# conradludgate/rustyguard

Hardware: AMD Instinct MI355X
Metric: GiB/s + Mpkt/s device-resident ChaCha20-Poly1305 seal/open, 1/2/4/8 MI355X (higher is better)
Workload: dtype u32; 1 GPU; cfg2: 64 Ki packets x 1500 B, one session key, seal then open, 1 MI355X; packets_per_gpu=65536, payload_bytes_per_packet=1504, wire_bytes_per_gpu=100663296, sessions=1, parallelism=split1 (no collective), split=1, wg_per_cu=auto

## Files before the change

rustyguard_amd/csrc/rg_internal.h:

```cpp
#pragma once
#include <hip/hip_ext.h>
#include <hip/hip_runtime.h>
#include <stdint.h>

#include "../../include/rg_aead.h"

namespace rg {

constexpr uint32_t kMaxPayload = 1u << 20;

struct SealArgs {
    const uint32_t *keys;
    const uint32_t *receivers;
    const rg_pkt_desc *desc;
    const uint64_t *counters;
    uint8_t *buf;
    uint64_t buf_len;
    uint8_t *status;
    uint64_t *dbg;
    uint32_t nkeys;
    uint32_t n;
};

struct OpenArgs {
    const uint32_t *keys;
    const rg_pkt_desc *desc;
    uint8_t *buf;
    uint64_t buf_len;
    uint8_t *status;
    uint64_t *counters_out;
    uint64_t *dbg;
    uint32_t nkeys;
    uint32_t n;
};

struct MacArgs {
    const uint32_t *keys;
    uint32_t key_len;
    uint32_t nkeys;
    uint32_t which;
    uint32_t n;
    const rg_pkt_desc *desc;
    const uint8_t *buf;
    uint64_t buf_len;
    uint8_t *status;
    uint32_t *key_out;
    uint32_t *key_state;
};
hipError_t launch_mac_verify(const MacArgs &a, hipStream_t s);

struct WorkspaceCursor {
    uint64_t at = 0;
    uint64_t take(uint64_t bytes) {
        const uint64_t o = at;
        at += (bytes + 255) & ~255ull;
        return o;
    }
    uint64_t total() const { return at ? at : 256; }
};

constexpr uint32_t kReplayTile = 2048;
struct ReplayLayout {
    uint64_t rdesc;
    uint64_t hash;
    uint64_t order[2];
    uint64_t hist;
    uint64_t agg_val;
    uint64_t agg_flag;
    uint64_t lf;
    uint64_t ctr;
    uint64_t widx;
    uint64_t undo;
    uint64_t ustatus;
    uint64_t udesc;
    uint64_t total;
    uint64_t hash_cap;
    uint32_t nblk;
    uint32_t passes;
};
inline ReplayLayout replay_layout(uint64_t n, uint32_t nwin) {
    ReplayLayout L{};
    if (n > 0xFFFFFFFFull) return L;
    WorkspaceCursor ws;
    L.hash_cap = 64;
    while (L.hash_cap < 2 * n) L.hash_cap <<= 1;
    L.nblk = (uint32_t)((n + kReplayTile - 1) / kReplayTile);
    for (uint32_t top = nwin ? nwin - 1 : 0; top; top >>= 8) ++L.passes;
    L.rdesc = ws.take(n * sizeof(rg_pkt_desc));
    L.hash = ws.take(L.hash_cap * 4);
    L.order[0] = ws.take(L.passes > 0 ? n * 4 : 0);
    L.order[1] = ws.take(L.passes > 1 ? n * 4 : 0);
    L.hist = ws.take(L.passes > 0 ? 256ull * L.nblk * 4 : 0);
    L.agg_val = ws.take((uint64_t)L.nblk * 8);
    L.agg_flag = ws.take((uint64_t)L.nblk * 4);
    L.lf = ws.take(n * 8);
    L.ctr = ws.take(n * 8);
    L.widx = ws.take(n * 4);
    L.undo = ws.take(n);
    L.ustatus = ws.take(n);
    L.udesc = ws.take(n * sizeof(rg_pkt_desc));
    L.total = ws.total();
    return L;
}

struct DeviceGuard {
    int dev = -1;
    DeviceGuard() { (void)hipGetDevice(&dev); }
    ~DeviceGuard() {
        if (dev >= 0) (void)hipSetDevice(dev);
    }
    DeviceGuard(const DeviceGuard &) = delete;
    DeviceGuard &operator=(const DeviceGuard &) = delete;
};

struct GeneralJob {
    uint32_t key[8];
    uint32_t nonce[3];
    uint32_t decrypt;
    uint32_t xchacha;
    uint32_t hnonce[4];
    uint64_t aad_off;
    uint64_t aad_len;
    uint64_t payload_off;
    uint64_t payload_len;
    uint64_t tag_off;
    uint32_t status;
    uint32_t pad_;
};

struct Launch {
    int lanes;
    int cus;
    int wg_per_cu;
    int debug_mode;
    int staged_g;
    hipEvent_t done;
};

#define RG_LAUNCH(done, kernel, grid, block, lds, stream, ...)                                              \
    do {                                                                                                   \
        if (done) hipExtLaunchKernelGGL(kernel, grid, block, lds, stream, nullptr, done, 0u, __VA_ARGS__); \
        else hipLaunchKernelGGL(kernel, grid, block, lds, stream, __VA_ARGS__);                            \
    } while (0)
constexpr uint32_t kLdsPerCu = 160u * 1024u;

constexpr uint32_t kClasses = 37;
__host__ __device__ __forceinline__ uint32_t class_hi(uint32_t c) {
    if (c <= 16) return c;
    const uint32_t j = c - 17;
    return (j & 1u) ? (1u << (j / 2 + 5)) : (3u << (j / 2 + 3));
}
__device__ __forceinline__ uint32_t class_of(uint32_t chunks) {
    if (chunks <= 16) return chunks;
    uint32_t c = 17;
    while (c < kClasses - 1 && class_hi(c) < chunks) ++c;
    return c;
}

struct TilePlan {
    const uint32_t *counts;
    const uint32_t *lists;
    uint32_t cap;
    uint32_t target_lanes;
    uint32_t fixed_k;
    uint32_t *classes_out;
    uint32_t *sched;
    uint32_t simds;
    uint32_t *gq;
};

hipError_t launch_plan(const rg_pkt_desc *desc, uint32_t n, bool open, const TilePlan &tp, hipStream_t s);
hipError_t launch_tiles(const SealArgs *sa, const OpenArgs *oa, int G, const TilePlan &tp, const Launch &L,
                        hipStream_t s);
hipError_t prepare_tile_kernels();
constexpr uint32_t kSchedWords = 128;
constexpr uint32_t kSchedStart = 4, kSchedLg = 44, kSchedCnt = 84;
static_assert(kSchedCnt + kClasses <= kSchedWords, "schedule words");

constexpr int kTargets = 6;
__device__ __forceinline__ void schedule_classes(uint32_t *counts, uint32_t *sched, uint32_t simds,
                                                 uint32_t *classes_out) {
    __shared__ uint32_t s_lg[kTargets][64], s_start[kTargets][64], s_est[kTargets], s_total[kTargets];
    __shared__ float s_sum[kTargets];
    const uint32_t c = threadIdx.x & 63, v = threadIdx.x >> 6;
    const uint32_t cnt =
        c < kClasses ? __hip_atomic_load(&counts[c], __ATOMIC_RELAXED, __HIP_MEMORY_SCOPE_AGENT) : 0;
    const uint32_t chunks = c < kClasses ? class_hi(c) : 0;
    const uint64_t used = __ballot(cnt > 0);
    float work = 0.0f;
    for (uint64_t m = used; m; m &= m - 1) {
        const int j = __ffsll((unsigned long long)m) - 1;
        work += (float)(uint32_t)__builtin_amdgcn_readlane((int)cnt, j) * (float)(1 + class_hi((uint32_t)j));
    }
    const uint32_t S = simds ? simds : 1;
    const float mean = work / (64.0f * (float)S);
    constexpr float kF[kTargets] = {1.0f, 1.25f, 1.5f, 2.0f, 3.0f, 0.0f};
    for (uint32_t k = v; k < (uint32_t)kTargets; k += 4) {
        const float tf = kF[k] > 0.0f ? ceilf(mean * kF[k]) : 65535.0f;
        const uint32_t target = tf < 2.0f ? 2u : tf > 65535.0f ? 65535u : (uint32_t)tf;
        uint32_t lg = 0;
        while (lg < 6 && 1 + ((chunks + (1u << lg) - 1) >> lg) > target) ++lg;
        const uint32_t tiles = cnt ? (uint32_t)((((uint64_t)cnt << lg) + 63) >> 6) : 0;
        const uint32_t w = cnt ? 1 + ((chunks + (1u << lg) - 1) >> lg) + (lg ? 1 : 0) : 0;
        uint32_t start = 0, total = 0;
        float sum = 0.0f;
        for (uint64_t m = used; m; m &= m - 1) {
            const int j = __ffsll((unsigned long long)m) - 1;
            const uint32_t wj = (uint32_t)__builtin_amdgcn_readlane((int)w, j);
            const uint32_t tj = (uint32_t)__builtin_amdgcn_readlane((int)tiles, j);
            if (wj > w || (wj == w && (uint32_t)j > c)) start += tj;
            total += tj;
            sum += (float)tj * (float)wj;
        }
        uint32_t est0 = 0, est1 = 0;
        for (uint32_t t = 0, m = 0; t < total; t += S, ++m) {
            const uint32_t a = t + (m & 1u ? S - 1 : 0), b = t + (m & 1u ? 0 : S - 1);
            const uint64_t ha = __ballot(tiles > 0 && start <= a && a < start + tiles);
            const uint64_t hb = __ballot(tiles > 0 && start <= b && b < start + tiles);
            if (ha) est0 += (uint32_t)__builtin_amdgcn_readlane((int)w, __ffsll((unsigned long long)ha) - 1);
            if (hb) est1 += (uint32_t)__builtin_amdgcn_readlane((int)w, __ffsll((unsigned long long)hb) - 1);
        }
        const uint32_t est = est0 > est1 ? est0 : est1;
        s_lg[k][c] = lg;
        s_start[k][c] = start;
        if (c == 0) {
            s_est[k] = est;
            s_sum[k] = sum;
            s_total[k] = total;
        }
    }
    __syncthreads();
    if (v != 0) return;
    uint32_t best = 0;
    for (uint32_t k = 1; k < (uint32_t)kTargets; ++k)
        if (s_est[k] < s_est[best] || (s_est[k] == s_est[best] && s_sum[k] < s_sum[best])) best = k;
    if (c < kClasses) {
        __hip_atomic_store(&counts[c], 0u, __ATOMIC_RELAXED, __HIP_MEMORY_SCOPE_AGENT);
        sched[kSchedStart + c] = s_start[best][c];
        sched[kSchedLg + c] = s_lg[best][c];
        sched[kSchedCnt + c] = cnt;
    }
    if (c == 0) {
        sched[2] = s_total[best];
        if (classes_out) *reinterpret_cast<volatile uint32_t *>(classes_out) = (uint32_t)__popcll(used);
    }
}

struct PipePlan {
    uint32_t *counts;
    const uint32_t *lists;
    uint32_t cap;
    uint32_t *sched;
    uint32_t *classes_out;
    uint32_t simds;
};
hipError_t launch_pipe(const SealArgs *sa, const OpenArgs *oa, const Launch &L, const PipePlan *plan,
                       hipStream_t s);

constexpr uint32_t kFlatGroup = 1024;
hipError_t launch_flat(const SealArgs *sa, const OpenArgs *oa, bool balance, uint4 *junk, int cus, hipStream_t s,
                       hipEvent_t done = nullptr);
uint32_t flat_junk_bytes(int cus);
hipError_t prepare_flat_kernels();
hipError_t prepare_pipe_kernels(int max_wg[2]);
hipError_t launch_rx_resolve(const rg_pkt_desc *desc, uint32_t n, const uint8_t *buf, uint64_t buf_len,
                             const rg_rx_entry *table, uint32_t cap, rg_pkt_desc *out, uint32_t *key_out,
                             hipStream_t s);
__host__ __device__ __forceinline__ uint32_t rx_slot(uint32_t receiver, uint32_t cap) {
    return cap > 1 ? (receiver * 0x9E3779B1u) >> (32 - __builtin_ctz(cap)) : 0u;
}
hipError_t launch_general(GeneralJob *jobs, uint32_t njobs, uint8_t *arena, hipStream_t s);
hipError_t launch_bind_keys(const rg_pkt_desc *in, const uint32_t *key_idx, uint32_t n, rg_pkt_desc *out,
                            hipStream_t s);
hipError_t launch_undo_gather(const rg_pkt_desc *rd, const uint64_t *ctr, const uint32_t *idx, uint32_t m,
                              rg_pkt_desc *out, uint64_t *ctr_out, hipStream_t s);
hipError_t launch_synth_fill(const rg_pkt_desc *desc, const uint32_t *inner_len, uint32_t n, uint8_t *buf,
                             uint64_t buf_len, uint64_t seed, hipStream_t s);

constexpr uint32_t kCtlCounts = 0;
constexpr uint32_t kCtlSched = 64;
constexpr uint32_t kCtlPool = 192;
constexpr uint32_t kCtlWords = 256;
static_assert(kCtlCounts + kClasses + 1 <= kCtlSched && kCtlSched + kSchedWords <= kCtlPool &&
                  kCtlPool + 33 <= kCtlWords, "control block layout");
hipError_t launch_preset(uint8_t *status, uint32_t n, uint32_t *ctl, uint32_t done_init, uint32_t pool_init,
                         hipStream_t s);

}
```

rustyguard_amd/csrc/rg_pipe.hip:

```cpp
#include "rg_device.h"
#include "rg_internal.h"

namespace rg {

struct Chunk {
    uint4 q0, q1, q2, q3;
};

constexpr int kDepth = 3;

typedef unsigned v4u __attribute__((ext_vector_type(4)));
template <int NT> __device__ __forceinline__ uint4 ld16(const uint4 *p) {
    if constexpr (NT & 1) {
        const v4u v = __builtin_nontemporal_load(reinterpret_cast<const v4u *>(p));
        return make_uint4(v.x, v.y, v.z, v.w);
    } else return *p;
}
template <int NT> __device__ __forceinline__ void st16(uint4 *p, const uint4 &x) {
    if constexpr (NT & 4) return;
    else if constexpr (NT & 2) {
        const v4u v = {x.x, x.y, x.z, x.w};
        __builtin_nontemporal_store(v, reinterpret_cast<v4u *>(p));
    } else *p = x;
}
template <int MODE> constexpr int mode_nt() { return MODE == 7 ? 4 : (MODE >= 4 && MODE <= 6) ? MODE - 3 : 0; }

template <int NT = 0>
__device__ __forceinline__ void load_chunk(Chunk &c, const uint4 *pl, uint32_t t, uint32_t last) {
    const uint32_t b = 4 * t;
    c.q0 = ld16<NT>(pl + min(b + 0, last));
    c.q1 = ld16<NT>(pl + min(b + 1, last));
    c.q2 = ld16<NT>(pl + min(b + 2, last));
    c.q3 = ld16<NT>(pl + min(b + 3, last));
}

__device__ __forceinline__ void absorb_chunk(Acc &h, const Chunk &c, const Mul &r, uint32_t cnt) {
    acc_block_pred(h, c.q0, r, cnt > 0);
    acc_block_pred(h, c.q1, r, cnt > 1);
    acc_block_pred(h, c.q2, r, cnt > 2);
    acc_block_pred(h, c.q3, r, cnt > 3);
}

constexpr uint32_t kPipeLinesFlag = 4u;
constexpr uint32_t kRingBytes = 64u * 256u;
typedef __attribute__((address_space(3))) v4u lds_u4;
__device__ __forceinline__ v4u to_v4(const uint4 &a) { return v4u{a.x, a.y, a.z, a.w}; }
__device__ __forceinline__ uint32_t ring_g(uint32_t p) { return (p & 1u) ^ (((p >> 1) & 1u) * 10u) ^ (((p >> 2) & 1u) * 4u); }

struct Ring {
    lds_u4 *wr;
    lds_u4 *rd;
    uint32_t fo[2][4];
    uint32_t self;
    uint64_t base;
    __amdgpu_buffer_rsrc_t rs;
    uint32_t gw, gr;
};

__device__ __forceinline__ bool frame_window(const uint8_t *frame, uint32_t len, uint64_t &base) {
    const uint64_t f = reinterpret_cast<uint64_t>(frame);
    const uint64_t f0 = uniform_u64(f);
    const int64_t dlt = (int64_t)(f - f0);
    const bool near = dlt > -(int64_t)(1u << 30) && dlt < (int64_t)(1u << 30);
    if (__ballot(!near) != 0) return false;
    const uint32_t v = (uint32_t)(dlt + (int64_t)(1u << 30));
    const uint32_t vmax = lane63(wave_scan_max(v)), vmin = 0x7FFFFFFFu - lane63(wave_scan_max(0x7FFFFFFFu - v));
    if ((uint64_t)(vmax - vmin) + len >= (1ull << 31)) return false;
    base = f0 + (uint64_t)vmin - (1ull << 30);
    return true;
}

__device__ __forceinline__ Ring make_ring(uint8_t *frame, uint64_t base) {
    extern __shared__ __attribute__((aligned(16))) uint8_t pipe_lds[];
    const uint32_t lane = threadIdx.x & 63;
    lds_u4 *lb = (lds_u4 *)(pipe_lds + (threadIdx.x >> 6) * kRingBytes);
    Ring R;
    R.wr = lb + 16 * lane;
    R.gw = ring_g(lane);
    R.rd = lb + 16 * (lane >> 3);
    R.gr = ring_g(lane >> 3);
    R.self = (uint32_t)(reinterpret_cast<uint64_t>(frame) - base);
    R.base = base;
    R.rs = __builtin_amdgcn_make_buffer_rsrc(reinterpret_cast<void *>(base), (short)0, 0x7FFFFFFF, 0x00020000);
#pragma unroll
    for (int h = 0; h < 2; ++h)
#pragma unroll
        for (int q = 0; q < 4; ++q)
            R.fo[h][q] = (uint32_t)__shfl((int)R.self, 32 * h + 8 * q + (int)(lane >> 3)) + 16 * (lane & 7u);
    return R;
}

__device__ __forceinline__ Ring pin_window(const Ring &R) {
    Ring o = R;
    o.base = uniform_u64(R.base);
    o.rs = __builtin_amdgcn_make_buffer_rsrc(reinterpret_cast<void *>(o.base), (short)0, 0x7FFFFFFF, 0x00020000);
    return o;
}

#ifndef RG_TAIL_CP
#define RG_TAIL_CP 0
#endif
constexpr int kTailCp = RG_TAIL_CP;

template <int CP = 0> __device__ __forceinline__ void frame_store(const Ring &R, uint32_t off, const uint4 &x) {
    __builtin_amdgcn_raw_buffer_store_b128(to_v4(x), R.rs, (int)(R.self + off), 0, CP);
}

__device__ __forceinline__ void ring_put(const Ring &R, uint32_t t, const uint4 &a, const uint4 &b, const uint4 &c,
                                         const uint4 &d) {
    const uint32_t sw = (4 * (t & 3u)) ^ R.gw;
    R.wr[sw ^ 0] = to_v4(a);
    R.wr[sw ^ 1] = to_v4(b);
    R.wr[sw ^ 2] = to_v4(c);
    R.wr[sw ^ 3] = to_v4(d);
}

struct Ring4 {
    v4u v[4];
};
__device__ __forceinline__ Ring4 ring_get(const Ring &R, uint32_t k, uint32_t h) {
    const uint32_t lane = threadIdx.x & 63;
    const uint32_t set = (2 * k + ((lane >> 2) & 1u)) & 3u;
    const lds_u4 *r = R.rd + 512 * h + ((4 * set + (lane & 3u)) ^ R.gr);
    Ring4 o;
#pragma unroll
    for (int q = 0; q < 4; ++q) o.v[q] = r[128 * q];
    return o;
}

template <bool MASK = false, int CP = 0>
__device__ __forceinline__ void ring_store(const Ring &R, const Ring4 &x, uint32_t k, uint32_t h, uint32_t nblk = 0) {
    if constexpr (MASK) {
        const uint32_t lane = threadIdx.x & 63;
        if (((lane >> 2) & 1u) && 2 * k + 1 >= nblk) return;
    }
#pragma unroll
    for (int q = 0; q < 4; ++q)
        __builtin_amdgcn_raw_buffer_store_b128(x.v[q], R.rs, (int)((h ? R.fo[1][q] : R.fo[0][q]) + 128 * k), 0, CP);
}

template <bool OPEN, bool ABSORB, bool TAIL, int MODE = 0, bool LINES = false, bool FLUSH = false>
__device__ __forceinline__ void pipe_step(uint4 *pl, const Stream &st, const Mul &r, Acc &h, Chunk &pi, Chunk &buf,
                                          uint4 &prev, bool &have_prev, uint32_t t, uint32_t nb, uint32_t c0,
                                          const Ring &R) {
    uint32_t ks[16];
    static_assert(!FLUSH || (LINES && ABSORB && !TAIL), "flush steps");
    Ring4 fl;
    if constexpr (FLUSH) {
        wave_sync();
        fl = ring_get(R, (t - 2) >> 1, t & 1u);
    }
    if constexpr (MODE == 2) {
#pragma unroll
        for (int i = 0; i < 16; ++i) ks[i] = t * 16 + i;
        h.h0 ^= pi.q0.x ^ pi.q1.y ^ pi.q2.z ^ pi.q3.w;
    } else stream_block_hooked(st, c0 + t + 1, ks, [&](int dr) {
        if constexpr (OPEN) {
            const uint32_t bl = TAIL ? nb & 3u : 4u;
            if (dr == 1) acc_block_pred(h, buf.q0, r, bl > 0);
            if (dr == 3) acc_block_pred(h, buf.q1, r, bl > 1);
            if (dr == 5) acc_block_pred(h, buf.q2, r, bl > 2);
            if (dr == 7) acc_block_pred(h, buf.q3, r, bl > 3);
            if (dr % 2 == 1) pin_acc(h);
        } else if constexpr (ABSORB) {
            if (dr == 1) acc_block(h, pi.q0, r);
            if (dr == 3) acc_block(h, pi.q1, r);
            if (dr == 5) acc_block(h, pi.q2, r);
            if (dr == 7) acc_block(h, pi.q3, r);
            if (dr % 2 == 1) pin_acc(h);
        }
    });
    Chunk x = {xor4(buf.q0, ks + 0), xor4(buf.q1, ks + 4), xor4(buf.q2, ks + 8), xor4(buf.q3, ks + 12)};
    uint4 *dst = pl + 4 * t;
    if constexpr (MODE == 1) {
        pi = x;
        buf.q0.x += t; buf.q1.y ^= t; buf.q2.z += h.h0; buf.q3.w ^= t;
        return;
    }
    constexpr int NT = mode_nt<MODE>();
    if constexpr (LINES && !TAIL) {
        ring_put(R, t, prev, x.q0, x.q1, x.q2);
        if constexpr (FLUSH) ring_store(R, fl, MODE == 8 ? ((t - 2) >> 1) & 1u : (t - 2) >> 1, t & 1u);
        prev = x.q3;
        have_prev = true;
    } else if constexpr (TAIL) {
        const uint32_t cnt = nb & 3u;
        if constexpr (LINES) {
            const uint32_t o = 16 + 64 * t;
            if (have_prev) frame_store<kTailCp>(R, o - 16, prev);
            frame_store<kTailCp>(R, o, x.q0);
            if (cnt > 1) frame_store<kTailCp>(R, o + 16, x.q1);
            if (cnt > 2) frame_store<kTailCp>(R, o + 32, x.q2);
        } else {
            if (have_prev) st16<NT>(dst - 1, prev);
            st16<NT>(dst + 0, x.q0);
            if (cnt > 1) st16<NT>(dst + 1, x.q1);
            if (cnt > 2) st16<NT>(dst + 2, x.q2);
        }
        have_prev = false;
    } else {
        if constexpr (ABSORB) st16<NT>(dst - 1, prev);
        else if (have_prev) st16<NT>(dst - 1, prev);
        st16<NT>(dst + 0, x.q0);
        st16<NT>(dst + 1, x.q1);
        st16<NT>(dst + 2, x.q2);
        prev = x.q3;
        have_prev = true;
    }
    if constexpr (!OPEN) pi = x;
    if constexpr (!TAIL) load_chunk<NT & 1>(buf, pl, t + kDepth, nb - 1);
}

template <bool OPEN, int MODE = 0, bool LINES = false>
__device__ __forceinline__ Acc pipe_pass(uint4 *pl, const Stream &st, const Mul &r, uint32_t nb, uint32_t c0,
                                         Chunk &b0, Chunk &b1, Chunk &b2, uint4 head, bool has_head, const Ring &R0) {
    const Ring R = LINES ? pin_window(R0) : R0;
    const uint32_t F = nb >> 2, bl = nb & 3u;
    Acc h = {0, 0, 0, 0, 0};
    Chunk pi = {};
    uint4 prev = head;
    bool have_prev = has_head;
    uint32_t pending = 0;
    if constexpr (LINES) wave_sync();
    if (F > 0) {
        pipe_step<OPEN, false, false, MODE, LINES>(pl, st, r, h, pi, b0, prev, have_prev, 0, nb, c0, R);
        uint32_t t = 1;
        if constexpr (LINES) {
            if (F > 1) pipe_step<OPEN, true, false, MODE, true>(pl, st, r, h, pi, b1, prev, have_prev, 1, nb, c0, R);
            for (t = 2; t + 2 < F; t += 3) {
                pipe_step<OPEN, true, false, MODE, true, true>(pl, st, r, h, pi, b2, prev, have_prev, t, nb, c0, R);
                pipe_step<OPEN, true, false, MODE, true, true>(pl, st, r, h, pi, b0, prev, have_prev, t + 1, nb, c0, R);
                pipe_step<OPEN, true, false, MODE, true, true>(pl, st, r, h, pi, b1, prev, have_prev, t + 2, nb, c0, R);
            }
            if (t < F) pipe_step<OPEN, true, false, MODE, true, true>(pl, st, r, h, pi, b2, prev, have_prev, t, nb, c0, R);
            if (t + 1 < F)
                pipe_step<OPEN, true, false, MODE, true, true>(pl, st, r, h, pi, b0, prev, have_prev, t + 1, nb, c0, R);
            wave_sync();
            for (uint32_t m = F >= 2 ? F - 2 : 0; m < 2 * ((F + 1) >> 1); ++m)
                ring_store<true, kTailCp>(R, ring_get(R, m >> 1, m & 1u), MODE == 8 ? (m >> 1) & 1u : m >> 1, m & 1u,
                                          F);
        } else {
            for (; t + 2 < F; t += 3) {
                pipe_step<OPEN, true, false, MODE, false>(pl, st, r, h, pi, b1, prev, have_prev, t, nb, c0, R);
                pipe_step<OPEN, true, false, MODE, false>(pl, st, r, h, pi, b2, prev, have_prev, t + 1, nb, c0, R);
                pipe_step<OPEN, true, false, MODE, false>(pl, st, r, h, pi, b0, prev, have_prev, t + 2, nb, c0, R);
            }
            if (t < F) pipe_step<OPEN, true, false, MODE, false>(pl, st, r, h, pi, b1, prev, have_prev, t, nb, c0, R);
            if (t + 1 < F) pipe_step<OPEN, true, false, MODE, false>(pl, st, r, h, pi, b2, prev, have_prev, t + 1, nb, c0, R);
        }
        pending = 4;
    }
    if (bl > 0) {
        const uint32_t k = F % kDepth;
        Chunk bp = {k == 1 ? b1.q0 : k == 2 ? b2.q0 : b0.q0, k == 1 ? b1.q1 : k == 2 ? b2.q1 : b0.q1,
                    k == 1 ? b1.q2 : k == 2 ? b2.q2 : b0.q2, k == 1 ? b1.q3 : k == 2 ? b2.q3 : b0.q3};
        if (F > 0) pipe_step<OPEN, true, true, MODE, LINES>(pl, st, r, h, pi, bp, prev, have_prev, F, nb, c0, R);
        else pipe_step<OPEN, false, true, MODE, LINES>(pl, st, r, h, pi, bp, prev, have_prev, F, nb, c0, R);
        pending = bl;
    }
    if constexpr (LINES) {
        if (have_prev) frame_store<kTailCp>(R, 64 * F, prev);
    } else if (have_prev && MODE != 1) st16<mode_nt<MODE>()>(pl + 4 * F - 1, prev);
    if constexpr (!OPEN) absorb_chunk(h, pi, r, pending);
    return h;
}

__device__ __forceinline__ void pipe_tag(Acc h, const Mul &r, uint32_t P, const uint32_t *s, uint32_t tag[4]) {
    acc_add(h, 0, 0, P, 0, 1);
    acc_mul(h, r);
    acc_finish(h, s[0], s[1], s[2], s[3], tag);
}

struct Seg {
    uint32_t c0, nb, after;
};

__device__ __forceinline__ Seg make_seg(uint32_t nb, uint32_t j, uint32_t G) {
    const uint32_t C = (nb + 3) >> 2, L = (C + G - 1) / G;
    const uint32_t c0 = min(j * L, C), c1 = min(c0 + L, C);
    const uint32_t b0 = min(4 * c0, nb), b1 = min(4 * c1, nb);
    return {c0, b1 - b0, nb - b1};
}

__device__ __forceinline__ uint32_t wave_max_u32(uint32_t v) {
#pragma unroll
    for (int o = 32; o >= 1; o >>= 1) v = max(v, (uint32_t)__shfl_xor((int)v, o));
    return v;
}

__device__ __forceinline__ Acc combine_segments(Acc h, const Mul &r, uint32_t after, uint32_t G) {
    if (G == 1) return h;
    const uint32_t bits = 32 - __clz((int)wave_max_u32(after));
    if (bits > 0) {
        Acc x = {1, 0, 0, 0, 0};
        for (int b = (int)bits - 1; b >= 0; --b) {
            Acc sq = x;
            acc_sqr_gen(sq);
            Acc xr = sq;
            acc_mul(xr, r);
            const bool bit = (after >> b) & 1u;
            x.h0 = bit ? xr.h0 : sq.h0; x.h1 = bit ? xr.h1 : sq.h1; x.h2 = bit ? xr.h2 : sq.h2;
            x.h3 = bit ? xr.h3 : sq.h3; x.h4 = bit ? xr.h4 : sq.h4;
        }
        acc_mul_gen(h, make_gen(x));
    }
    for (uint32_t o = 1; o < G; o <<= 1) {
        Acc other;
        other.h0 = (uint32_t)__shfl_xor((int)h.h0, (int)o);
        other.h1 = (uint32_t)__shfl_xor((int)h.h1, (int)o);
        other.h2 = (uint32_t)__shfl_xor((int)h.h2, (int)o);
        other.h3 = (uint32_t)__shfl_xor((int)h.h3, (int)o);
        other.h4 = (uint32_t)__shfl_xor((int)h.h4, (int)o);
        acc_add_acc(h, other);
        acc_fold(h);
    }
    return h;
}

template <int MODE>
__device__ __forceinline__ void pipe_seal_packet(const SealArgs &a, uint32_t i, const rg_pkt_desc &d, uint32_t j,
                                                 uint32_t G, bool lines_ok) {
    const uint32_t P = d.len;
    const bool valid = d.key_idx < a.nkeys && (P & 15u) == 0 && (d.offset & 15u) == 0 && P <= kMaxPayload &&
                       d.offset <= a.buf_len && P + 32 <= a.buf_len - d.offset;
    bool lines = false;
    if constexpr (MODE == 0 || MODE == 8)
        lines = lines_ok && G == 1 && __ballot(valid && P == uniform_u32(P)) == ~0ull;
    uint64_t wbase = 0;
    if (lines) lines = frame_window(a.buf + d.offset, P + 32, wbase);
    if (!valid) {
        if (a.status && j == 0) a.status[i] = d.key_idx == RG_KEY_SKIP ? RG_PKT_REJECTED : RG_PKT_INVALID;
        return;
    }
    uint8_t *frame = a.buf + d.offset;
    const uint32_t nb = P >> 4;
    const Seg sg = make_seg(nb, j, G);
    uint4 *pl = reinterpret_cast<uint4 *>(frame + 16) + (sg.nb ? 4 * sg.c0 : 0);
    Chunk b0, b1, b2;
    if constexpr (MODE == 1) {
        b0 = {make_uint4(i, 1, 2, 3), make_uint4(4, i, 6, 7), make_uint4(8, 9, i, 11), make_uint4(12, 13, 14, i)};
        b1 = b0;
        b2 = b0;
    } else {
        constexpr int NT = mode_nt<MODE>() & 1;
        load_chunk<NT>(b0, pl, 0, sg.nb ? sg.nb - 1 : 0);
        load_chunk<NT>(b1, pl, 1, sg.nb ? sg.nb - 1 : 0);
        load_chunk<NT>(b2, pl, 2, sg.nb ? sg.nb - 1 : 0);
    }
    const Key8 key = load_key(a.keys, d.key_idx);
    const uint64_t ctr = a.counters[i];
    const uint32_t n1 = (uint32_t)ctr, n2 = (uint32_t)(ctr >> 32);
    const Stream stm = make_stream(key, 0u, n1, n2);
    uint32_t ks[16];
    stream_block(stm, 0, ks);
    const Mul r = make_mul(ks[0], ks[1], ks[2], ks[3]);
    const bool head = a.receivers != nullptr && j == 0;
    uint4 hdr = make_uint4(4u, head ? a.receivers[d.key_idx] : 0u, n1, n2);
    Acc h;
    Ring R{};
    if (lines) {
        if (!head) hdr = *reinterpret_cast<const uint4 *>(frame);
        R = make_ring(frame, wbase);
        h = pipe_pass<false, MODE, true>(pl, stm, r, sg.nb, sg.c0, b0, b1, b2, hdr, true, R);
    } else {
        h = pipe_pass<false, MODE, false>(pl, stm, r, sg.nb, sg.c0, b0, b1, b2, hdr, head, Ring{});
    }
    h = combine_segments(h, r, sg.after, G);
    if (j != 0) return;
    uint32_t tag[4];
    pipe_tag(h, r, P, ks + 4, tag);
    const uint4 tagv = make_uint4(tag[0], tag[1], tag[2], tag[3]);
    if (lines) frame_store<kTailCp>(pin_window(R), 16 + P, tagv);
    else *reinterpret_cast<uint4 *>(frame + 16 + P) = tagv;
    if (a.status) a.status[i] = RG_PKT_OK;
}

__device__ __forceinline__ void pipe_open_packet(const OpenArgs &a, uint32_t i, const rg_pkt_desc &d, uint32_t j,
                                                 uint32_t G, bool lines_ok) {
    const uint32_t W = d.len;
    uint32_t st;
    if (d.key_idx == RG_KEY_SKIP) st = RG_PKT_REJECTED;
    else if ((d.offset & 15u) != 0) st = RG_PKT_UNALIGNED;
    else if (d.key_idx >= a.nkeys || W > kMaxPayload + 32 || d.offset > a.buf_len || W > a.buf_len - d.offset ||
             W < 4)
        st = RG_PKT_INVALID;
    else st = 0xFF;
    uint8_t *frame = a.buf + d.offset;
    const bool desc_ok = st == 0xFF;
    const bool go = desc_ok && W >= 32 && (W & 15u) == 0;
    const uint32_t P = go ? W - 32 : 0;
    const uint32_t nb = P >> 4;
    const Seg sg = make_seg(nb, j, G);
    uint4 *safe = const_cast<uint4 *>(reinterpret_cast<const uint4 *>(a.desc + i));
    uint4 *pl = go ? reinterpret_cast<uint4 *>(frame + 16) + (sg.nb ? 4 * sg.c0 : 0) : safe;
    const uint4 hdr = *(desc_ok ? reinterpret_cast<const uint4 *>(frame) : safe);
    Chunk b0, b1, b2;
    load_chunk(b0, pl, 0, sg.nb ? sg.nb - 1 : 0);
    load_chunk(b1, pl, 1, sg.nb ? sg.nb - 1 : 0);
    load_chunk(b2, pl, 2, sg.nb ? sg.nb - 1 : 0);
    const uint4 want = *(go ? reinterpret_cast<const uint4 *>(frame + 16 + P) : safe);
    const Key8 key = load_key(a.keys, go ? d.key_idx : 0);
    uint64_t ctr = 0;
    if (desc_ok) {
        if (hdr.x != 4u) st = hdr.x - 1u < 3u ? RG_PKT_NOT_DATA : RG_PKT_INVALID;
        else if ((W & 15u) != 0 || W < 16) st = RG_PKT_INVALID;
        else {
            ctr = ((uint64_t)hdr.w << 32) | hdr.z;
            if (W < 32) st = RG_PKT_DECRYPT_ERR;
        }
    }
    bool lines = lines_ok && G == 1 && __ballot(st == 0xFF && W == uniform_u32(W)) == ~0ull;
    uint64_t wbase = 0;
    if (lines) lines = frame_window(frame, W, wbase);
    if (st != 0xFF) {
        if (j == 0) {
            a.status[i] = (uint8_t)st;
            if (a.counters_out) a.counters_out[i] = ctr;
        }
        return;
    }
    const uint32_t n1 = (uint32_t)ctr, n2 = (uint32_t)(ctr >> 32);
    const Stream stm = make_stream(key, 0u, n1, n2);
    uint32_t ks[16];
    stream_block(stm, 0, ks);
    const Mul r = make_mul(ks[0], ks[1], ks[2], ks[3]);
    Acc h;
    Ring Ro{};
    if (lines) Ro = make_ring(frame, wbase);
    if (lines) h = pipe_pass<true, 0, true>(pl, stm, r, sg.nb, sg.c0, b0, b1, b2, hdr, true, Ro);
    else h = pipe_pass<true, 0, false>(pl, stm, r, sg.nb, sg.c0, b0, b1, b2, make_uint4(0, 0, 0, 0), false, Ring{});
    h = combine_segments(h, r, sg.after, G);
    uint32_t tag[4];
    pipe_tag(h, r, P, ks + 4, tag);
    const uint32_t diff = (tag[0] ^ want.x) | (tag[1] ^ want.y) | (tag[2] ^ want.z) | (tag[3] ^ want.w);
    if (__ballot(diff != 0)) {
        wave_sync();
        restore_forged(diff != 0, key, n1, n2, pl, sg.c0, sg.nb);
    }
    if (j == 0) {
        a.status[i] = diff == 0 ? RG_PKT_OK : RG_PKT_DECRYPT_ERR;
        if (a.counters_out) a.counters_out[i] = ctr;
    }
}

#if RG_DIAG
__device__ __forceinline__ void pipe_stamp(uint64_t *dbg, uint64_t t0, uint64_t r0, const uint64_t marks[3]) {
    const uint64_t t1 = __builtin_amdgcn_s_memtime(), r1 = __builtin_amdgcn_s_memrealtime();
    if ((threadIdx.x & 63) == 0) {
        uint64_t *o = dbg + 8ull * (blockIdx.x * (blockDim.x / 64) + threadIdx.x / 64);
        o[0] = t1 - t0;
        o[1] = marks[0] ? marks[0] - r0 : 0;
        o[2] = marks[1] ? marks[1] - r0 : 0;
        o[3] = ((uint64_t)(uint32_t)__builtin_amdgcn_s_getreg(0xF814) << 32) | (uint32_t)__builtin_amdgcn_s_getreg(0xF804);
        o[4] = r0;
        o[5] = marks[2] ? marks[2] - t0 : 0;
        o[6] = 1;
        o[7] = r1 - r0;
    }
}
#endif

template <class Body>
__device__ __forceinline__ void pipe_walk(uint32_t n, uint32_t lg0, const PipePlan &pp, const rg_pkt_desc *desc,
                                          bool stamp, uint64_t marks[3], Body &&body) {
    const uint32_t lane = threadIdx.x & 63;
    const bool planned = pp.counts != nullptr;
    uint32_t my_cnt = 0, my_start = 0, my_lg = 0, my_tiles = 0, S = 1, simd = 0, ntiles = 0;
    uint64_t total, first, stride;
    if (planned) {
        my_cnt = lane < kClasses ? pp.sched[kSchedCnt + lane] : 0;
        my_start = lane < kClasses ? pp.sched[kSchedStart + lane] : 0;
        my_lg = lane < kClasses ? pp.sched[kSchedLg + lane] : 0;
        my_tiles = (uint32_t)((((uint64_t)my_cnt << my_lg) + 63) / 64);
        S = pp.simds ? pp.simds : 1;
        const uint32_t slot = blockIdx.x * (blockDim.x / 64) + threadIdx.x / 64;
        simd = slot % S;
        ntiles = pp.sched[2];
        total = (ntiles + S - 1) / S;
        first = slot / S;
        stride = gridDim.x * (blockDim.x / 64) / S;
    } else {
        total = (uint64_t)n << lg0;
        first = blockIdx.x * 256 + threadIdx.x;
        stride = (uint64_t)gridDim.x * 256;
    }
    struct Unit {
        uint32_t i, j, lg;
        bool live;
    };
    auto locate = [&](uint64_t it, uint32_t &list_pos) -> Unit {
        Unit o;
        list_pos = 0;
        if (planned) {
            const uint32_t tile = (uint32_t)it * S + ((it & 1u) ? S - 1 - simd : simd);
            const uint64_t hit = __ballot(lane < kClasses && my_start <= tile && tile < my_start + my_tiles);
            const uint32_t c = uniform_u32((uint32_t)(__ffsll((unsigned long long)hit) - 1));
            o.lg = uniform_u32((uint32_t)__shfl((int)my_lg, (int)c));
            const uint32_t u = (tile - uniform_u32((uint32_t)__shfl((int)my_start, (int)c))) * 64 + lane;
            const uint32_t p = u >> o.lg;
            o.live = tile < ntiles && p < uniform_u32((uint32_t)__shfl((int)my_cnt, (int)c));
            o.j = u & ((1u << o.lg) - 1);
            list_pos = o.live ? c * pp.cap + p : 0;
            o.i = 0;
        } else {
            o.lg = lg0;
            o.live = it < total;
            o.j = (uint32_t)it & ((1u << lg0) - 1);
            o.i = o.live ? (uint32_t)(it >> lg0) : 0;
        }
        return o;
    };
    if (first >= total) return;
    uint32_t q0, q1;
    Unit cur = locate(first, q0), nxt = locate(first + stride, q1);
    if (planned) {
        cur.i = pp.lists[q0];
        nxt.i = pp.lists[q1];
    }
    rg_pkt_desc dcur = desc[cur.live ? cur.i : 0];
    for (uint64_t it = first; it < total; it += stride) {
        uint32_t q2;
        Unit far = locate(it + 2 * stride, q2);
        if (planned) far.i = pp.lists[q2];
        const rg_pkt_desc dnxt = desc[nxt.live ? nxt.i : 0];
        if (stamp && it == first) marks[2] = __builtin_amdgcn_s_memtime();
        if (cur.live) body(cur.i, dcur, cur.j, 1u << cur.lg);
        if (stamp) {
            const uint64_t now = __builtin_amdgcn_s_memrealtime();
            if (it == first) marks[0] = now;
            else if (it == first + stride) marks[1] = now;
        }
        cur = nxt;
        nxt = far;
        dcur = dnxt;
    }
}

template <int MODE> __global__ __launch_bounds__(256) void pipe_seal_kernel(SealArgs a, uint32_t flags, PipePlan pp) {
    uint64_t marks[3] = {0, 0, 0};
    const bool lines = (flags & kPipeLinesFlag) != 0;
#if RG_DIAG
    const uint64_t t0 = __builtin_amdgcn_s_memtime(), r0 = __builtin_amdgcn_s_memrealtime();
    const bool stamp = a.dbg != nullptr;
#else
    constexpr bool stamp = false;
#endif
    pipe_walk(a.n, flags & 3u, pp, a.desc, stamp, marks, [=](uint32_t i, const rg_pkt_desc &d, uint32_t j, uint32_t G) {
        pipe_seal_packet<MODE>(a, i, d, j, G, lines);
    });
#if RG_DIAG
    if (stamp) pipe_stamp(a.dbg, t0, r0, marks);
#endif
}

__global__ __launch_bounds__(256) void pipe_open_kernel(OpenArgs a, uint32_t flags, PipePlan pp) {
    uint64_t marks[3] = {0, 0, 0};
    const bool lines = (flags & kPipeLinesFlag) != 0;
#if RG_DIAG
    const uint64_t t0 = __builtin_amdgcn_s_memtime(), r0 = __builtin_amdgcn_s_memrealtime();
    const bool stamp = a.dbg != nullptr;
#else
    constexpr bool stamp = false;
#endif
    pipe_walk(a.n, flags & 3u, pp, a.desc, stamp, marks, [=](uint32_t i, const rg_pkt_desc &d, uint32_t j, uint32_t G) {
        pipe_open_packet(a, i, d, j, G, lines);
    });
#if RG_DIAG
    if (stamp) pipe_stamp(a.dbg, t0, r0, marks);
#endif
}

static void pipe_grid(uint64_t units, const Launch &L, uint32_t &blocks, uint32_t &lds) {
    const uint64_t want = (units + 255) / 256;
    const uint64_t cap = (uint64_t)L.cus * (uint64_t)L.wg_per_cu;
    blocks = (uint32_t)(want < cap || cap == 0 ? want : cap);
    lds = L.wg_per_cu > 0 ? (kLdsPerCu / L.wg_per_cu) & ~255u : 0;
}

hipError_t launch_pipe(const SealArgs *sa, const OpenArgs *oa, const Launch &L, const PipePlan *plan,
                       hipStream_t s) {
    const uint32_t n = sa ? sa->n : oa->n;
    if (n == 0) return hipSuccess;
    const uint32_t lg = L.lanes >= 4 ? 2 : L.lanes == 2 ? 1 : 0;
    PipePlan pp{};
    uint32_t blocks, lds;
    if (plan) {
        pp = *plan;
        const uint32_t wg = (uint32_t)(L.wg_per_cu > 0 ? L.wg_per_cu : 1);
        blocks = (uint32_t)(L.cus > 0 ? L.cus : 1) * wg;
        lds = (kLdsPerCu / wg) & ~255u;
        if (pp.simds == 0 || ((uint64_t)blocks * 4) % pp.simds != 0) return hipErrorInvalidValue;
    } else {
        pipe_grid((uint64_t)n << lg, L, blocks, lds);
    }
    const uint32_t fl = lg | (lds >= 4 * kRingBytes ? kPipeLinesFlag : 0u);
    if (oa) {
        RG_LAUNCH(L.done, pipe_open_kernel, dim3(blocks), dim3(256), lds, s, *oa, fl, pp);
        return hipGetLastError();
    }
#if RG_DIAG
    switch (L.debug_mode) {
    case 1: hipLaunchKernelGGL(pipe_seal_kernel<1>, dim3(blocks), dim3(256), lds, s, *sa, fl, pp); return hipGetLastError();
    case 2: hipLaunchKernelGGL(pipe_seal_kernel<2>, dim3(blocks), dim3(256), lds, s, *sa, fl, pp); return hipGetLastError();
    case 4: hipLaunchKernelGGL(pipe_seal_kernel<4>, dim3(blocks), dim3(256), lds, s, *sa, fl, pp); return hipGetLastError();
    case 5: hipLaunchKernelGGL(pipe_seal_kernel<5>, dim3(blocks), dim3(256), lds, s, *sa, fl, pp); return hipGetLastError();
    case 6: hipLaunchKernelGGL(pipe_seal_kernel<6>, dim3(blocks), dim3(256), lds, s, *sa, fl, pp); return hipGetLastError();
    case 7: hipLaunchKernelGGL(pipe_seal_kernel<7>, dim3(blocks), dim3(256), lds, s, *sa, fl, pp); return hipGetLastError();
    case 8: hipLaunchKernelGGL(pipe_seal_kernel<8>, dim3(blocks), dim3(256), lds, s, *sa, fl, pp); return hipGetLastError();
    default: break;
    }
#endif
    RG_LAUNCH(L.done, pipe_seal_kernel<0>, dim3(blocks), dim3(256), lds, s, *sa, fl, pp);
    return hipGetLastError();
}

hipError_t prepare_pipe_kernels(int max_wg[2]) {
    const void *f[2] = {(const void *)pipe_seal_kernel<0>, (const void *)pipe_open_kernel};
    for (int w = 0; w < 2; ++w) {
        hipError_t e = hipFuncSetAttribute(f[w], hipFuncAttributeMaxDynamicSharedMemorySize, (int)kLdsPerCu);
        if (e != hipSuccess) return e;
        int nb = 0;
        e = hipOccupancyMaxActiveBlocksPerMultiprocessor(&nb, f[w], 256, 0);
        if (e != hipSuccess) return e;
        max_wg[w] = nb;
    }
#if RG_DIAG
    const void *d[7] = {(const void *)pipe_seal_kernel<1>, (const void *)pipe_seal_kernel<2>,
                        (const void *)pipe_seal_kernel<4>, (const void *)pipe_seal_kernel<5>,
                        (const void *)pipe_seal_kernel<6>, (const void *)pipe_seal_kernel<7>,
                        (const void *)pipe_seal_kernel<8>};
    for (const void *k : d) {
        hipError_t e = hipFuncSetAttribute(k, hipFuncAttributeMaxDynamicSharedMemorySize, (int)kLdsPerCu);
        if (e != hipSuccess) return e;
    }
#endif
    return hipSuccess;
}

}
```

Baseline: 1385 GiB/s.

## Load frame-aligned 64B blocks including header and tag in the pipe loop

Reindexes the pipelined seal/open loads so each 64-byte chunk is aligned to the frame start rather than the payload start. The 16-byte header and the trailing tag now arrive as part of the prefetched chunks, replacing separate header and tag loads and the carried 'prev' register. Open gets the header and tag from the chunk buffers, using lane shuffles when a packet is split across lanes. The intent is fully aligned line-sized accesses and fewer scattered loads. The cost is more complex index bookkeeping and some extra shuffles.

```diff
diff --git a/rustyguard_amd/csrc/rg_internal.h b/rustyguard_amd/csrc/rg_internal.h
--- a/rustyguard_amd/csrc/rg_internal.h
+++ b/rustyguard_amd/csrc/rg_internal.h
@@ -257,6 +257,22 @@
 hipError_t launch_pipe(const SealArgs *sa, const OpenArgs *oa, const Launch &L, const PipePlan *plan,
                        hipStream_t s);
 
+struct Seg {
+    uint32_t c0, nb, after;
+};
+__host__ __device__ inline Seg make_seg(uint32_t nb, uint32_t j, uint32_t G) {
+    const uint32_t C = (nb + 3) >> 2, L = (C + G - 1) / G;
+    const uint32_t c0 = j * L < C ? j * L : C, c1 = c0 + L < C ? c0 + L : C;
+    const uint32_t b0 = 4 * c0 < nb ? 4 * c0 : nb, b1 = 4 * c1 < nb ? 4 * c1 : nb;
+    return {c0, b1 - b0, nb - b1};
+}
+__host__ __device__ inline uint32_t pipe_piece(uint32_t blk, uint32_t i, uint32_t hi) {
+    const uint32_t p = 4 * blk + i;
+    return p < hi ? p : hi;
+}
+__host__ __device__ inline uint32_t pipe_full_steps(uint32_t nb) { return nb >> 2; }
+__host__ __device__ inline uint32_t pipe_last_blocks(uint32_t nb) { return nb & 3u; }
+
 constexpr uint32_t kFlatGroup = 1024;
 hipError_t launch_flat(const SealArgs *sa, const OpenArgs *oa, bool balance, uint4 *junk, int cus, hipStream_t s,
                        hipEvent_t done = nullptr);
diff --git a/rustyguard_amd/csrc/rg_pipe.hip b/rustyguard_amd/csrc/rg_pipe.hip
--- a/rustyguard_amd/csrc/rg_pipe.hip
+++ b/rustyguard_amd/csrc/rg_pipe.hip
@@ -26,12 +26,11 @@
 template <int MODE> constexpr int mode_nt() { return MODE == 7 ? 4 : (MODE >= 4 && MODE <= 6) ? MODE - 3 : 0; }
 
 template <int NT = 0>
-__device__ __forceinline__ void load_chunk(Chunk &c, const uint4 *pl, uint32_t t, uint32_t last) {
-    const uint32_t b = 4 * t;
-    c.q0 = ld16<NT>(pl + min(b + 0, last));
-    c.q1 = ld16<NT>(pl + min(b + 1, last));
-    c.q2 = ld16<NT>(pl + min(b + 2, last));
-    c.q3 = ld16<NT>(pl + min(b + 3, last));
+__device__ __forceinline__ void load_block(Chunk &c, const uint4 *fr, uint32_t blk, uint32_t hi) {
+    c.q0 = ld16<NT>(fr + pipe_piece(blk, 0, hi));
+    c.q1 = ld16<NT>(fr + pipe_piece(blk, 1, hi));
+    c.q2 = ld16<NT>(fr + pipe_piece(blk, 2, hi));
+    c.q3 = ld16<NT>(fr + pipe_piece(blk, 3, hi));
 }
 
 __device__ __forceinline__ void absorb_chunk(Acc &h, const Chunk &c, const Mul &r, uint32_t cnt) {
@@ -140,9 +139,9 @@
 }
 
 template <bool OPEN, bool ABSORB, bool TAIL, int MODE = 0, bool LINES = false, bool FLUSH = false>
-__device__ __forceinline__ void pipe_step(uint4 *pl, const Stream &st, const Mul &r, Acc &h, Chunk &pi, Chunk &buf,
-                                          uint4 &prev, bool &have_prev, uint32_t t, uint32_t nb, uint32_t c0,
-                                          const Ring &R) {
+__device__ __forceinline__ void pipe_step(uint4 *fb, const uint4 *fr, const Stream &st, const Mul &r, Acc &h, Chunk &pi,
+                                          Chunk &buf, Chunk &nxt, bool first, uint32_t t, uint32_t nb, uint32_t c0,
+                                          uint32_t hi, const Ring &R) {
     uint32_t ks[16];
     static_assert(!FLUSH || (LINES && ABSORB && !TAIL), "flush steps");
     Ring4 fl;
@@ -156,11 +155,11 @@
         h.h0 ^= pi.q0.x ^ pi.q1.y ^ pi.q2.z ^ pi.q3.w;
     } else stream_block_hooked(st, c0 + t + 1, ks, [&](int dr) {
         if constexpr (OPEN) {
-            const uint32_t bl = TAIL ? nb & 3u : 4u;
-            if (dr == 1) acc_block_pred(h, buf.q0, r, bl > 0);
-            if (dr == 3) acc_block_pred(h, buf.q1, r, bl > 1);
-            if (dr == 5) acc_block_pred(h, buf.q2, r, bl > 2);
-            if (dr == 7) acc_block_pred(h, buf.q3, r, bl > 3);
+            const uint32_t bl = TAIL ? pipe_last_blocks(nb) : 4u;
+            if (dr == 1) acc_block_pred(h, buf.q1, r, bl > 0);
+            if (dr == 3) acc_block_pred(h, buf.q2, r, bl > 1);
+            if (dr == 5) acc_block_pred(h, buf.q3, r, bl > 2);
+            if (dr == 7) acc_block_pred(h, nxt.q0, r, bl > 3);
             if (dr % 2 == 1) pin_acc(h);
         } else if constexpr (ABSORB) {
             if (dr == 1) acc_block(h, pi.q0, r);
@@ -170,8 +169,12 @@
             if (dr % 2 == 1) pin_acc(h);
         }
     });
-    Chunk x = {xor4(buf.q0, ks + 0), xor4(buf.q1, ks + 4), xor4(buf.q2, ks + 8), xor4(buf.q3, ks + 12)};
-    uint4 *dst = pl + 4 * t;
+    Chunk x = {xor4(buf.q1, ks + 0), xor4(buf.q2, ks + 4), xor4(buf.q3, ks + 8), buf.q0};
+    if constexpr (!TAIL) {
+        x.q3 = xor4(nxt.q0, ks + 12);
+        nxt.q0 = x.q3;
+    }
+    uint4 *dst = fb + 4 * t;
     if constexpr (MODE == 1) {
         pi = x;
         buf.q0.x += t; buf.q1.y ^= t; buf.q2.z += h.h0; buf.q3.w ^= t;
@@ -179,88 +182,83 @@
     }
     constexpr int NT = mode_nt<MODE>();
     if constexpr (LINES && !TAIL) {
-        ring_put(R, t, prev, x.q0, x.q1, x.q2);
+        ring_put(R, t, buf.q0, x.q0, x.q1, x.q2);
         if constexpr (FLUSH) ring_store(R, fl, MODE == 8 ? ((t - 2) >> 1) & 1u : (t - 2) >> 1, t & 1u);
-        prev = x.q3;
-        have_prev = true;
     } else if constexpr (TAIL) {
-        const uint32_t cnt = nb & 3u;
+        const uint32_t cnt = pipe_last_blocks(nb);
+        const bool have = ABSORB || first;
         if constexpr (LINES) {
-            const uint32_t o = 16 + 64 * t;
-            if (have_prev) frame_store<kTailCp>(R, o - 16, prev);
-            frame_store<kTailCp>(R, o, x.q0);
-            if (cnt > 1) frame_store<kTailCp>(R, o + 16, x.q1);
-            if (cnt > 2) frame_store<kTailCp>(R, o + 32, x.q2);
+            const uint32_t o = 64 * t;
+            if (have) frame_store<kTailCp>(R, o, buf.q0);
+            frame_store<kTailCp>(R, o + 16, x.q0);
+            if (cnt > 1) frame_store<kTailCp>(R, o + 32, x.q1);
+            if (cnt > 2) frame_store<kTailCp>(R, o + 48, x.q2);
         } else {
-            if (have_prev) st16<NT>(dst - 1, prev);
-            st16<NT>(dst + 0, x.q0);
-            if (cnt > 1) st16<NT>(dst + 1, x.q1);
-            if (cnt > 2) st16<NT>(dst + 2, x.q2);
-        }
-        have_prev = false;
+            if (have) st16<NT>(dst + 0, buf.q0);
+            st16<NT>(dst + 1, x.q0);
+            if (cnt > 1) st16<NT>(dst + 2, x.q1);
+            if (cnt > 2) st16<NT>(dst + 3, x.q2);
+        }
     } else {
-        if constexpr (ABSORB) st16<NT>(dst - 1, prev);
-        else if (have_prev) st16<NT>(dst - 1, prev);
-        st16<NT>(dst + 0, x.q0);
-        st16<NT>(dst + 1, x.q1);
-        st16<NT>(dst + 2, x.q2);
-        prev = x.q3;
-        have_prev = true;
+        if constexpr (ABSORB) st16<NT>(dst + 0, buf.q0);
+        else if (first) st16<NT>(dst + 0, buf.q0);
+        st16<NT>(dst + 1, x.q0);
+        st16<NT>(dst + 2, x.q1);
+        st16<NT>(dst + 3, x.q2);
     }
     if constexpr (!OPEN) pi = x;
-    if constexpr (!TAIL) load_chunk<NT & 1>(buf, pl, t + kDepth, nb - 1);
+    if constexpr (!TAIL) load_block<NT & 1>(buf, fr, c0 + t + kDepth, hi);
 }
 
 template <bool OPEN, int MODE = 0, bool LINES = false>
-__device__ __forceinline__ Acc pipe_pass(uint4 *pl, const Stream &st, const Mul &r, uint32_t nb, uint32_t c0,
-                                         Chunk &b0, Chunk &b1, Chunk &b2, uint4 head, bool has_head, const Ring &R0) {
+__device__ __forceinline__ Acc pipe_pass(const uint4 *fr, const Stream &st, const Mul &r, uint32_t nb, uint32_t c0,
+                                         uint32_t hi, Chunk &b0, Chunk &b1, Chunk &b2, bool first, const Ring &R0) {
     const Ring R = LINES ? pin_window(R0) : R0;
-    const uint32_t F = nb >> 2, bl = nb & 3u;
+    const uint32_t F = pipe_full_steps(nb), bl = pipe_last_blocks(nb);
+    uint4 *fb = const_cast<uint4 *>(fr) + 4 * c0;
     Acc h = {0, 0, 0, 0, 0};
     Chunk pi = {};
-    uint4 prev = head;
-    bool have_prev = has_head;
     uint32_t pending = 0;
     if constexpr (LINES) wave_sync();
     if (F > 0) {
-        pipe_step<OPEN, false, false, MODE, LINES>(pl, st, r, h, pi, b0, prev, have_prev, 0, nb, c0, R);
+        pipe_step<OPEN, false, false, MODE, LINES>(fb, fr, st, r, h, pi, b0, b1, first, 0, nb, c0, hi, R);
         uint32_t t = 1;
         if constexpr (LINES) {
-            if (F > 1) pipe_step<OPEN, true, false, MODE, true>(pl, st, r, h, pi, b1, prev, have_prev, 1, nb, c0, R);
+            if (F > 1) pipe_step<OPEN, true, false, MODE, true>(fb, fr, st, r, h, pi, b1, b2, first, 1, nb, c0, hi, R);
             for (t = 2; t + 2 < F; t += 3) {
-                pipe_step<OPEN, true, false, MODE, true, true>(pl, st, r, h, pi, b2, prev, have_prev, t, nb, c0, R);
-                pipe_step<OPEN, true, false, MODE, true, true>(pl, st, r, h, pi, b0, prev, have_prev, t + 1, nb, c0, R);
-                pipe_step<OPEN, true, false, MODE, true, true>(pl, st, r, h, pi, b1, prev, have_prev, t + 2, nb, c0, R);
+                pipe_step<OPEN, true, false, MODE, true, true>(fb, fr, st, r, h, pi, b2, b0, first, t, nb, c0, hi, R);
+                pipe_step<OPEN, true, false, MODE, true, true>(fb, fr, st, r, h, pi, b0, b1, first, t + 1, nb, c0, hi, R);
+                pipe_step<OPEN, true, false, MODE, true, true>(fb, fr, st, r, h, pi, b1, b2, first, t + 2, nb, c0, hi, R);
             }
-            if (t < F) pipe_step<OPEN, true, false, MODE, true, true>(pl, st, r, h, pi, b2, prev, have_prev, t, nb, c0, R);
+            if (t < F) pipe_step<OPEN, true, false, MODE, true, true>(fb, fr, st, r, h, pi, b2, b0, first, t, nb, c0, hi, R);
             if (t + 1 < F)
-                pipe_step<OPEN, true, false, MODE, true, true>(pl, st, r, h, pi, b0, prev, have_prev, t + 1, nb, c0, R);
+                pipe_step<OPEN, true, false, MODE, true, true>(fb, fr, st, r, h, pi, b0, b1, first, t + 1, nb, c0, hi, R);
             wave_sync();
             for (uint32_t m = F >= 2 ? F - 2 : 0; m < 2 * ((F + 1) >> 1); ++m)
                 ring_store<true, kTailCp>(R, ring_get(R, m >> 1, m & 1u), MODE == 8 ? (m >> 1) & 1u : m >> 1, m & 1u,
                                           F);
         } else {
             for (; t + 2 < F; t += 3) {
-                pipe_step<OPEN, true, false, MODE, false>(pl, st, r, h, pi, b1, prev, have_prev, t, nb, c0, R);
-                pipe_step<OPEN, true, false, MODE, false>(pl, st, r, h, pi, b2, prev, have_prev, t + 1, nb, c0, R);
-                pipe_step<OPEN, true, false, MODE, false>(pl, st, r, h, pi, b0, prev, have_prev, t + 2, nb, c0, R);
+                pipe_step<OPEN, true, false, MODE, false>(fb, fr, st, r, h, pi, b1, b2, first, t, nb, c0, hi, R);
+                pipe_step<OPEN, true, false, MODE, false>(fb, fr, st, r, h, pi, b2, b0, first, t + 1, nb, c0, hi, R);
+                pipe_step<OPEN, true, false, MODE, false>(fb, fr, st, r, h, pi, b0, b1, first, t + 2, nb, c0, hi, R);
             }
-            if (t < F) pipe_step<OPEN, true, false, MODE, false>(pl, st, r, h, pi, b1, prev, have_prev, t, nb, c0, R);
-            if (t + 1 < F) pipe_step<OPEN, true, false, MODE, false>(pl, st, r, h, pi, b2, prev, have_prev, t + 1, nb, c0, R);
+            if (t < F) pipe_step<OPEN, true, false, MODE, false>(fb, fr, st, r, h, pi, b1, b2, first, t, nb, c0, hi, R);
+            if (t + 1 < F) pipe_step<OPEN, true, false, MODE, false>(fb, fr, st, r, h, pi, b2, b0, first, t + 1, nb, c0, hi, R);
         }
         pending = 4;
     }
+    const uint32_t k = F % kDepth;
+    Chunk bp = {k == 1 ? b1.q0 : k == 2 ? b2.q0 : b0.q0, k == 1 ? b1.q1 : k == 2 ? b2.q1 : b0.q1,
+                k == 1 ? b1.q2 : k == 2 ? b2.q2 : b0.q2, k == 1 ? b1.q3 : k == 2 ? b2.q3 : b0.q3};
     if (bl > 0) {
-        const uint32_t k = F % kDepth;
-        Chunk bp = {k == 1 ? b1.q0 : k == 2 ? b2.q0 : b0.q0, k == 1 ? b1.q1 : k == 2 ? b2.q1 : b0.q1,
-                    k == 1 ? b1.q2 : k == 2 ? b2.q2 : b0.q2, k == 1 ? b1.q3 : k == 2 ? b2.q3 : b0.q3};
-        if (F > 0) pipe_step<OPEN, true, true, MODE, LINES>(pl, st, r, h, pi, bp, prev, have_prev, F, nb, c0, R);
-        else pipe_step<OPEN, false, true, MODE, LINES>(pl, st, r, h, pi, bp, prev, have_prev, F, nb, c0, R);
+        if (F > 0) pipe_step<OPEN, true, true, MODE, LINES>(fb, fr, st, r, h, pi, bp, bp, first, F, nb, c0, hi, R);
+        else pipe_step<OPEN, false, true, MODE, LINES>(fb, fr, st, r, h, pi, bp, bp, first, F, nb, c0, hi, R);
         pending = bl;
-    }
-    if constexpr (LINES) {
-        if (have_prev) frame_store<kTailCp>(R, 64 * F, prev);
-    } else if (have_prev && MODE != 1) st16<mode_nt<MODE>()>(pl + 4 * F - 1, prev);
+    } else if (F > 0 || first) {
+        if constexpr (LINES) frame_store<kTailCp>(R, 64 * F, bp.q0);
+        else if constexpr (MODE != 1) st16<mode_nt<MODE>()>(fb + 4 * F, bp.q0);
+    }
     if constexpr (!OPEN) absorb_chunk(h, pi, r, pending);
     return h;
 }
@@ -271,16 +269,6 @@
     acc_finish(h, s[0], s[1], s[2], s[3], tag);
 }
 
-struct Seg {
-    uint32_t c0, nb, after;
-};
-
-__device__ __forceinline__ Seg make_seg(uint32_t nb, uint32_t j, uint32_t G) {
-    const uint32_t C = (nb + 3) >> 2, L = (C + G - 1) / G;
-    const uint32_t c0 = min(j * L, C), c1 = min(c0 + L, C);
-    const uint32_t b0 = min(4 * c0, nb), b1 = min(4 * c1, nb);
-    return {c0, b1 - b0, nb - b1};
-}
 
 __device__ __forceinline__ uint32_t wave_max_u32(uint32_t v) {
 #pragma unroll
@@ -335,7 +323,8 @@
     uint8_t *frame = a.buf + d.offset;
     const uint32_t nb = P >> 4;
     const Seg sg = make_seg(nb, j, G);
-    uint4 *pl = reinterpret_cast<uint4 *>(frame + 16) + (sg.nb ? 4 * sg.c0 : 0);
+    const uint4 *fr = reinterpret_cast<const uint4 *>(frame);
+    const uint32_t hi = nb + 1;
     Chunk b0, b1, b2;
     if constexpr (MODE == 1) {
         b0 = {make_uint4(i, 1, 2, 3), make_uint4(4, i, 6, 7), make_uint4(8, 9, i, 11), make_uint4(12, 13, 14, i)};
@@ -343,9 +332,9 @@
         b2 = b0;
     } else {
         constexpr int NT = mode_nt<MODE>() & 1;
-        load_chunk<NT>(b0, pl, 0, sg.nb ? sg.nb - 1 : 0);
-        load_chunk<NT>(b1, pl, 1, sg.nb ? sg.nb - 1 : 0);
-        load_chunk<NT>(b2, pl, 2, sg.nb ? sg.nb - 1 : 0);
+        load_block<NT>(b0, fr, sg.c0 + 0, hi);
+        load_block<NT>(b1, fr, sg.c0 + 1, hi);
+        load_block<NT>(b2, fr, sg.c0 + 2, hi);
     }
     const Key8 key = load_key(a.keys, d.key_idx);
     const uint64_t ctr = a.counters[i];
@@ -355,15 +344,14 @@
     stream_block(stm, 0, ks);
     const Mul r = make_mul(ks[0], ks[1], ks[2], ks[3]);
     const bool head = a.receivers != nullptr && j == 0;
-    uint4 hdr = make_uint4(4u, head ? a.receivers[d.key_idx] : 0u, n1, n2);
+    if (head) b0.q0 = make_uint4(4u, a.receivers[d.key_idx], n1, n2);
     Acc h;
     Ring R{};
     if (lines) {
-        if (!head) hdr = *reinterpret_cast<const uint4 *>(frame);
         R = make_ring(frame, wbase);
-        h = pipe_pass<false, MODE, true>(pl, stm, r, sg.nb, sg.c0, b0, b1, b2, hdr, true, R);
+        h = pipe_pass<false, MODE, true>(fr, stm, r, sg.nb, sg.c0, hi, b0, b1, b2, true, R);
     } else {
-        h = pipe_pass<false, MODE, false>(pl, stm, r, sg.nb, sg.c0, b0, b1, b2, hdr, head, Ring{});
+        h = pipe_pass<false, MODE, false>(fr, stm, r, sg.nb, sg.c0, hi, b0, b1, b2, head, Ring{});
     }
     h = combine_segments(h, r, sg.after, G);
     if (j != 0) return;
@@ -391,14 +379,20 @@
     const uint32_t P = go ? W - 32 : 0;
     const uint32_t nb = P >> 4;
     const Seg sg = make_seg(nb, j, G);
-    uint4 *safe = const_cast<uint4 *>(reinterpret_cast<const uint4 *>(a.desc + i));
-    uint4 *pl = go ? reinterpret_cast<uint4 *>(frame + 16) + (sg.nb ? 4 * sg.c0 : 0) : safe;
-    const uint4 hdr = *(desc_ok ? reinterpret_cast<const uint4 *>(frame) : safe);
+    const uint4 *safe = reinterpret_cast<const uint4 *>(a.desc + i);
+    const uint4 *fr = desc_ok ? reinterpret_cast<const uint4 *>(frame) : safe;
+    const uint32_t hi = go ? nb + 1 : 0;
+    uint4 *pl = reinterpret_cast<uint4 *>(frame + 16) + (sg.nb ? 4 * sg.c0 : 0);
     Chunk b0, b1, b2;
-    load_chunk(b0, pl, 0, sg.nb ? sg.nb - 1 : 0);
-    load_chunk(b1, pl, 1, sg.nb ? sg.nb - 1 : 0);
-    load_chunk(b2, pl, 2, sg.nb ? sg.nb - 1 : 0);
-    const uint4 want = *(go ? reinterpret_cast<const uint4 *>(frame + 16 + P) : safe);
+    load_block(b0, fr, sg.c0 + 0, hi);
+    load_block(b1, fr, sg.c0 + 1, hi);
+    load_block(b2, fr, sg.c0 + 2, hi);
+    uint4 hdr = b0.q0;
+    if (G > 1) {
+        const int l0 = (int)((threadIdx.x & 63u) & ~(G - 1));
+        hdr = make_uint4((uint32_t)__shfl((int)hdr.x, l0), (uint32_t)__shfl((int)hdr.y, l0),
+                         (uint32_t)__shfl((int)hdr.z, l0), (uint32_t)__shfl((int)hdr.w, l0));
+    }
     const Key8 key = load_key(a.keys, go ? d.key_idx : 0);
     uint64_t ctr = 0;
     if (desc_ok) {
@@ -427,9 +421,16 @@
     Acc h;
     Ring Ro{};
     if (lines) Ro = make_ring(frame, wbase);
-    if (lines) h = pipe_pass<true, 0, true>(pl, stm, r, sg.nb, sg.c0, b0, b1, b2, hdr, true, Ro);
-    else h = pipe_pass<true, 0, false>(pl, stm, r, sg.nb, sg.c0, b0, b1, b2, make_uint4(0, 0, 0, 0), false, Ring{});
+    if (lines) h = pipe_pass<true, 0, true>(fr, stm, r, sg.nb, sg.c0, hi, b0, b1, b2, true, Ro);
+    else h = pipe_pass<true, 0, false>(fr, stm, r, sg.nb, sg.c0, hi, b0, b1, b2, false, Ring{});
     h = combine_segments(h, r, sg.after, G);
+    const uint32_t kw = (pipe_full_steps(sg.nb) + 1) % kDepth;
+    uint4 want = kw == 1 ? b1.q0 : kw == 2 ? b2.q0 : b0.q0;
+    if (G > 1) {
+        const int ll = (int)((threadIdx.x & 63u) | (G - 1));
+        want = make_uint4((uint32_t)__shfl((int)want.x, ll), (uint32_t)__shfl((int)want.y, ll),
+                          (uint32_t)__shfl((int)want.z, ll), (uint32_t)__shfl((int)want.w, ll));
+    }
     uint32_t tag[4];
     pipe_tag(h, r, P, ks + 4, tag);
     const uint32_t diff = (tag[0] ^ want.x) | (tag[1] ^ want.y) | (tag[2] ^ want.z) | (tag[3] ^ want.w);
```

Result: slower. 1370 GiB/s (-1.1%).
